# ArchieGertsman/spark-sched-sim

Hardware: AMD Instinct MI355X
Metric: env-steps/sec at 4096 batched envs (TPC-H, 10 exec) (higher is better)
Workload: dtype int64+f64

## Files before the change

include/sss.h:

```cpp
#ifndef SSS_H
#define SSS_H
#include <stddef.h>
#include <stdint.h>

#ifdef __cplusplus
extern "C" {
#endif

typedef struct sss_handle sss_handle;

typedef struct sss_cfg {
  int32_t num_executors;
  int32_t job_arrival_cap;
  int32_t max_jobs;
  int32_t reserved;
  double job_arrival_rate;
  double moving_delay;
  double warmup_delay;
  double beta;
} sss_cfg;

typedef struct sss_dims {
  int32_t num_envs, num_executors, job_cap, stage_stride;
  int32_t node_cap;
// ... 24 lines not shown
  SSS_E_STALLED = 5,
  SSS_E_NO_DURATION = 6,
  SSS_E_INVARIANT = 7,
  SSS_E_NEED_RESET = 8,
  SSS_E_NO_LIMIT = 9,
  SSS_E_CAPACITY = 10
};

int sss_query_dims(const sss_cfg* cfg, const void* pack, size_t pack_bytes, int num_envs, sss_dims* out);

int sss_create(const sss_cfg* cfg, const void* pack, size_t pack_bytes, int num_envs, int device, sss_handle** out);

int sss_bind_buffers(sss_handle* h, const sss_buffers* buffers);

int sss_reset(sss_handle* h, const uint64_t* seeds_dev, const double* time_limits_dev, const uint8_t* mask_dev, void* stream);

#define SSS_SKIP_ENV (-2147483647 - 1)
int sss_step(sss_handle* h, const int32_t* stage_idx_dev, const int32_t* num_exec_dev, int auto_reset, uint64_t seed_stride, void* stream);

int sss_step_bounded(sss_handle* h, const int32_t* stage_idx_dev, const int32_t* num_exec_dev, int auto_reset, uint64_t seed_stride, int max_events,
                     uint8_t* ready_dev, void* stream);

int sss_policy(sss_handle* h, int policy, int param, int32_t* stage_idx_dev, int32_t* num_exec_dev, void* stream);

int sss_rollout(sss_handle* h, int policy, int param, int n_steps, int auto_reset, uint64_t seed_stride, void* stream);

typedef struct sss_decima_graph {
  const uint8_t* active_dev;
  const int64_t* node_off_dev;
  const int64_t* job_off_dev;
  const int64_t* edge_off_dev;
  float num_tasks_scale;
  float work_scale;
  float* x_dev;
  int64_t* node_obs_dev;
  int64_t* node_loc_dev;
  int64_t* node_job_dev;
  int64_t* sched_rank_dev;
  int32_t* gen_dev;
  uint32_t* node_recv_dev;
  uint8_t* stage_mask_dev;
  int64_t* src_dev;
  int64_t* dst_dev;
  int64_t* edge_obs_dev;
  uint32_t* edge_layers_dev;
  int64_t* job_obs_dev;
// ... 378 lines not shown
```

spark_sched_sim_amd/binding.py:

```python
from __future__ import annotations

import ctypes as C
import os.path as osp

CSRC = osp.join(osp.dirname(osp.abspath(__file__)), "csrc")
LIB_NAME = "libsss_hip.so"


class SssCfg(C.Structure):
    _fields_ = [("num_executors", C.c_int32), ("job_arrival_cap", C.c_int32), ("max_jobs", C.c_int32),
                ("reserved", C.c_int32), ("job_arrival_rate", C.c_double), ("moving_delay", C.c_double),
                ("warmup_delay", C.c_double), ("beta", C.c_double)]


class SssDims(C.Structure):
    _fields_ = [("num_envs", C.c_int32), ("num_executors", C.c_int32), ("job_cap", C.c_int32),
                ("stage_stride", C.c_int32), ("node_cap", C.c_int32), ("edge_cap", C.c_int32),
                ("obs_i32", C.c_int32), ("obs_f64", C.c_int32), ("state_bytes", C.c_int64),
                ("env_stride", C.c_int64), ("off_t_arrival", C.c_int64), ("off_t_completed", C.c_int64),
                ("off_jobs", C.c_int64), ("off_active", C.c_int64), ("off_dur_ring", C.c_int64),
                ("job_rec_bytes", C.c_int32), ("hdr_bytes", C.c_int32)]


class SssBuffers(C.Structure):
# ... 133 lines not shown
    _fields_ = [("t_dev", C.c_void_p), ("job_dev", C.c_void_p), ("count_dev", C.c_void_p), ("cap", C.c_int32), ("pad_", C.c_int32)]


class SssTimelineRenderArgs(C.Structure):
    _fields_ = [("env_ids_dev", C.c_void_p), ("n", C.c_int32), ("width", C.c_int32), ("height", C.c_int32), ("pad_", C.c_int32), ("rgb_dev", C.c_void_p)]


REWARD_WINDOW_CHUNK = 64


def reward_window_scratch(T: int, B: int) -> int:
    return ((T + REWARD_WINDOW_CHUNK - 1) // REWARD_WINDOW_CHUNK + 1) * B + 1


class SssArenaArray(C.Structure):
    _fields_ = [("src_dev", C.c_void_p), ("dst_dev", C.c_void_p), ("elem_bytes", C.c_int32), ("per_row", C.c_int32), ("kind", C.c_int32), ("shift", C.c_int32)]


class SssArenaArgs(C.Structure):
    _fields_ = [("n_arrays", C.c_int32), ("n_obs", C.c_int32), ("totals_dev", C.c_void_p), ("cursor_dev", C.c_void_p), ("capacity", C.c_int64 * 4),
                ("rows_hint", C.c_int64), ("arrays", SssArenaArray * 24)]


EXPORTS = ["sss_query_dims", "sss_create", "sss_bind_buffers", "sss_reset", "sss_step", "sss_step_bounded", "sss_policy", "sss_rollout",
           "sss_decima_graph_build", "sss_decima_layer_lists", "sss_prefix_rows", "sss_decima_policy", "sss_decima_sample", "sss_gnn_launch",
           "sss_linear_wgrad_scratch", "sss_linear_wgrad", "sss_mlp_supported", "sss_mlp_recompute_supported", "sss_mlp_split_supported", "sss_mlp_forward", "sss_mlp_backward", "sss_mlp_wgrad_scratch", "sss_mlp_backward_wgrad", "sss_mlp_wgrad_finish", "sss_collect_step", "sss_gnn_encode", "sss_rows_op", "sss_rows_concat", "sss_segment_categorical", "sss_bit_lists", "sss_arena_append", "sss_discounted_returns", "sss_sequence_baselines", "sss_reward_window_update", "sss_differential_returns", "sss_bind_timeline", "sss_timeline_render", "sss_last_error", "sss_destroy", "sss_abi_sizeof"]
POLICY_IDS = {"fair": 0, "fifo": 1, "hash": 2, "wfair": 3, "sjfcp": 4}
WFAIR_ALPHA_RANGE = (-4, 4)
ABI_STRUCTS = {"sss_cfg": SssCfg, "sss_dims": SssDims, "sss_buffers": SssBuffers, "sss_decima_graph": SssDecimaGraph, "sss_decima_lists": SssDecimaLists,
               "sss_bit_list_args": SssBitListArgs, "sss_gnn_args": SssGnnArgs, "sss_decima_policy_args": SssDecimaPolicyArgs,
               "sss_decima_sample_args": SssDecimaSampleArgs, "sss_gnn_encode_args": SssGnnEncodeArgs, "sss_collect_args": SssCollectArgs,
               "sss_mlp_args": SssMlpArgs, "sss_arena_array": SssArenaArray, "sss_arena_args": SssArenaArgs, "sss_returns_args": SssReturnsArgs,
               "sss_baseline_args": SssBaselineArgs, "sss_rows_args": SssRowsArgs, "sss_concat_part": SssConcatPart, "sss_concat_args": SssConcatArgs, "sss_segcat_args": SssSegcatArgs}
ABI_TAGGED_STRUCTS = {"sss_reward_window_args": SssRewardWindowArgs, "sss_diffret_args": SssDiffretArgs}
ABI_PLAIN_STRUCTS = {"sss_timeline": SssTimeline, "sss_timeline_render_args": SssTimelineRenderArgs}


def load_library(path: str | None = None) -> C.CDLL:
    path = path or osp.join(CSRC, LIB_NAME)
    if not osp.exists(path):
        raise RuntimeError(
            f"{path} not found: the HIP extension has not been built "
            "(run `python -c 'import __graft_entry__ as g; g.build()'` or spark_sched_sim_amd/build.py). "
            "There is no CPU fallback.")
    return C.CDLL(path)


class Binding:
    def __init__(self, lib: C.CDLL | None = None):
        self.lib = lib if lib is not None else load_library()
        L = self.lib
        L.sss_query_dims.argtypes = [C.POINTER(SssCfg), C.c_void_p, C.c_size_t, C.c_int, C.POINTER(SssDims)]
        L.sss_create.argtypes = [C.POINTER(SssCfg), C.c_void_p, C.c_size_t, C.c_int, C.c_int, C.POINTER(C.c_void_p)]
        L.sss_bind_buffers.argtypes = [C.c_void_p, C.POINTER(SssBuffers)]
        L.sss_reset.argtypes = [C.c_void_p, C.c_void_p, C.c_void_p, C.c_void_p, C.c_void_p]
        L.sss_step.argtypes = [C.c_void_p, C.c_void_p, C.c_void_p, C.c_int, C.c_uint64, C.c_void_p]
        L.sss_step_bounded.argtypes = [C.c_void_p, C.c_void_p, C.c_void_p, C.c_int, C.c_uint64, C.c_int, C.c_void_p, C.c_void_p]
        L.sss_policy.argtypes = [C.c_void_p, C.c_int, C.c_int, C.c_void_p, C.c_void_p, C.c_void_p]
        L.sss_rollout.argtypes = [C.c_void_p, C.c_int, C.c_int, C.c_int, C.c_int, C.c_uint64, C.c_void_p]
        L.sss_decima_graph_build.argtypes = [C.c_void_p, C.POINTER(SssDecimaGraph), C.c_void_p]
        L.sss_decima_layer_lists.argtypes = [C.c_int, C.POINTER(SssDecimaLists), C.c_void_p]
        L.sss_prefix_rows.argtypes = [C.c_void_p, C.c_int64, C.c_int64, C.c_void_p, C.c_int, C.c_int, C.c_void_p, C.c_void_p, C.c_void_p, C.c_void_p]
        L.sss_decima_policy.argtypes = [C.c_void_p, C.POINTER(SssDecimaPolicyArgs), C.c_void_p]
        L.sss_decima_sample.argtypes = [C.c_int, C.c_int, C.POINTER(SssDecimaSampleArgs), C.c_void_p]
        L.sss_gnn_launch.argtypes = [C.c_int, C.POINTER(SssGnnArgs), C.c_void_p]
        L.sss_linear_wgrad_scratch.argtypes = [C.c_int, C.c_int]
        L.sss_linear_wgrad_scratch.restype = C.c_int64
        L.sss_linear_wgrad.argtypes = [C.c_void_p, C.c_int64, C.c_void_p, C.c_int64, C.c_int64, C.c_int, C.c_int, C.c_void_p, C.c_void_p, C.c_void_p, C.c_void_p]
        L.sss_gnn_encode.argtypes = [C.POINTER(SssGnnEncodeArgs), C.c_void_p]
        L.sss_collect_step.argtypes = [C.POINTER(SssCollectArgs), C.c_int, C.c_void_p]
        L.sss_mlp_supported.argtypes = [C.c_int] * 5
        L.sss_mlp_recompute_supported.argtypes = [C.c_int]
        L.sss_mlp_split_supported.argtypes = [C.c_int]
        L.sss_mlp_forward.argtypes = [C.POINTER(SssMlpArgs), C.c_void_p]
        L.sss_mlp_backward.argtypes = [C.POINTER(SssMlpArgs), C.c_void_p]
        L.sss_mlp_wgrad_scratch.argtypes = [C.c_int]
        L.sss_mlp_wgrad_scratch.restype = C.c_int64
        L.sss_mlp_backward_wgrad.argtypes = [C.POINTER(SssMlpArgs), C.c_void_p, C.c_void_p]
        L.sss_mlp_wgrad_finish.argtypes = [C.c_int] + [C.c_void_p] * 8
        L.sss_discounted_returns.argtypes = [C.POINTER(SssReturnsArgs), C.c_void_p]
# ... 43 lines not shown
```

spark_sched_sim_amd/csrc/sss_hip_sim.hip:

```cpp
#include <hip/hip_runtime.h>

#include "sss_sim.h"
#include "sss_narrow.h"

#ifdef SSS_TIMELINE
#define SSS_LAUNCHER(name) sss_narrow_tl_launch_##name
#define SSS_TL_DISPATCH(call)
#else
#define SSS_LAUNCHER(name) sss_narrow_launch_##name
#define SSS_TL_DISPATCH(call) \
  if (a.tl.t) return sss_narrow_tl_launch_##call
int sss_narrow_hot_bytes() { return (int)sizeof(SssHot); }
int sss_narrow_static_lds_bytes() { return SSS_STATIC_LDS_BYTES; }
#endif

int SSS_LAUNCHER(reset)(const SssKernelArgs& a, int num_envs, const uint64_t* seeds, const double* tl, const uint8_t* mask, void* stream) {
  SSS_TL_DISPATCH(reset(a, num_envs, seeds, tl, mask, stream));
  hipLaunchKernelGGL(SSS_KNAME(sss_reset_kernel), dim3(num_envs), dim3(64), (size_t)a.P.pool_bytes, (hipStream_t)stream, a, seeds, tl, mask);
  return (int)hipGetLastError();
}
int SSS_LAUNCHER(step_bounded)(const SssKernelArgs& a, int num_envs, const int32_t* stage_idx, const int32_t* num_exec, int auto_reset, uint64_t seed_stride,
                                   int budget, uint8_t* ready, void* stream) {
  SSS_TL_DISPATCH(step_bounded(a, num_envs, stage_idx, num_exec, auto_reset, seed_stride, budget, ready, stream));
  hipLaunchKernelGGL(SSS_KNAME(sss_step_bounded_kernel), dim3(num_envs), dim3(64), (size_t)a.P.pool_bytes, (hipStream_t)stream, a, stage_idx, num_exec, auto_reset, seed_stride,
                     budget, ready);
  return (int)hipGetLastError();
}
int SSS_LAUNCHER(step)(const SssKernelArgs& a, int num_envs, const int32_t* stage_idx, const int32_t* num_exec, int auto_reset, uint64_t seed_stride,
                           void* stream) {
  SSS_TL_DISPATCH(step(a, num_envs, stage_idx, num_exec, auto_reset, seed_stride, stream));
  hipLaunchKernelGGL(SSS_KNAME(sss_step_kernel), dim3(num_envs), dim3(64), (size_t)a.P.pool_bytes, (hipStream_t)stream, a, stage_idx, num_exec, auto_reset, seed_stride);
  return (int)hipGetLastError();
}
#ifndef SSS_TIMELINE
int SSS_LAUNCHER(policy)(const SssKernelArgs& a, int num_envs, int policy, int param, int32_t* stage_idx, int32_t* num_exec, void* stream) {
  hipLaunchKernelGGL(SSS_KNAME(sss_policy_kernel), dim3(num_envs), dim3(64), (size_t)a.P.pool_bytes, (hipStream_t)stream, a, policy, param, stage_idx, num_exec);
  return (int)hipGetLastError();
}
#endif
int SSS_LAUNCHER(rollout)(const SssKernelArgs& a, int num_envs, int policy, int param, int n_steps, int auto_reset, uint64_t seed_stride, void* stream) {
  SSS_TL_DISPATCH(rollout(a, num_envs, policy, param, n_steps, auto_reset, seed_stride, stream));
  if (policy >= SSS_POLICY_WFAIR)
    hipLaunchKernelGGL(SSS_KNAME(sss_rollout_heur_kernel), dim3(num_envs), dim3(64), (size_t)a.P.pool_bytes, (hipStream_t)stream, a, policy, param, n_steps, auto_reset, seed_stride);
  else
    hipLaunchKernelGGL(SSS_KNAME(sss_rollout_kernel), dim3(num_envs), dim3(64), (size_t)a.P.pool_bytes, (hipStream_t)stream, a, policy, param, n_steps, auto_reset, seed_stride);
  return (int)hipGetLastError();
}

#if defined(SSS_EVPROF3) && !defined(SSS_TIMELINE)
extern "C" int sss_debug_prof(unsigned long long* out64) {
  if (hipMemcpyFromSymbol(out64, HIP_SYMBOL(g_prof3), sizeof(unsigned long long) * 96) != hipSuccess) return -1;
  static const unsigned long long zeros[96] = {0};
  return hipMemcpyToSymbol(HIP_SYMBOL(g_prof3), zeros, sizeof(zeros)) == hipSuccess ? 0 : -1;
// ... 6 lines not shown
```

spark_sched_sim_amd/csrc/sss_hip_wide.hip:

```cpp
#define SSS_WIDE 1
#include <hip/hip_runtime.h>

#include "sss_sim.h"
#include "sss_wide.h"

#ifdef SSS_TIMELINE
#define SSS_LAUNCHER(name) sss_wide_tl_launch_##name
#define SSS_TL_DISPATCH(call)
#else
#define SSS_LAUNCHER(name) sss_wide_launch_##name
#define SSS_TL_DISPATCH(call) \
  if (a.tl.t) return sss_wide_tl_launch_##call
int sss_wide_hot_bytes() { return (int)sizeof(SssHot); }
int sss_wide_static_lds_bytes() { return SSS_STATIC_LDS_BYTES; }
#endif

int SSS_LAUNCHER(reset)(const SssKernelArgs& a, int num_envs, const uint64_t* seeds, const double* tl, const uint8_t* mask, void* stream) {
  SSS_TL_DISPATCH(reset(a, num_envs, seeds, tl, mask, stream));
  hipLaunchKernelGGL(SSS_KNAME(sss_reset_kernel), dim3(num_envs), dim3(64), (size_t)a.P.pool_bytes, (hipStream_t)stream, a, seeds, tl, mask);
  return (int)hipGetLastError();
}
int SSS_LAUNCHER(step_bounded)(const SssKernelArgs& a, int num_envs, const int32_t* stage_idx, const int32_t* num_exec, int auto_reset, uint64_t seed_stride,
                                 int budget, uint8_t* ready, void* stream) {
  SSS_TL_DISPATCH(step_bounded(a, num_envs, stage_idx, num_exec, auto_reset, seed_stride, budget, ready, stream));
  hipLaunchKernelGGL(SSS_KNAME(sss_step_bounded_kernel), dim3(num_envs), dim3(64), (size_t)a.P.pool_bytes, (hipStream_t)stream, a, stage_idx, num_exec, auto_reset,
                     seed_stride, budget, ready);
  return (int)hipGetLastError();
}
int SSS_LAUNCHER(step)(const SssKernelArgs& a, int num_envs, const int32_t* stage_idx, const int32_t* num_exec, int auto_reset, uint64_t seed_stride,
                         void* stream) {
  SSS_TL_DISPATCH(step(a, num_envs, stage_idx, num_exec, auto_reset, seed_stride, stream));
  hipLaunchKernelGGL(SSS_KNAME(sss_step_kernel), dim3(num_envs), dim3(64), (size_t)a.P.pool_bytes, (hipStream_t)stream, a, stage_idx, num_exec, auto_reset, seed_stride);
  return (int)hipGetLastError();
}
#ifndef SSS_TIMELINE
int SSS_LAUNCHER(policy)(const SssKernelArgs& a, int num_envs, int policy, int param, int32_t* stage_idx, int32_t* num_exec, void* stream) {
  hipLaunchKernelGGL(SSS_KNAME(sss_policy_kernel), dim3(num_envs), dim3(64), (size_t)a.P.pool_bytes, (hipStream_t)stream, a, policy, param, stage_idx, num_exec);
  return (int)hipGetLastError();
}
#endif
int SSS_LAUNCHER(rollout)(const SssKernelArgs& a, int num_envs, int policy, int param, int n_steps, int auto_reset, uint64_t seed_stride, void* stream) {
  SSS_TL_DISPATCH(rollout(a, num_envs, policy, param, n_steps, auto_reset, seed_stride, stream));
  if (policy >= SSS_POLICY_WFAIR)
    hipLaunchKernelGGL(SSS_KNAME(sss_rollout_heur_kernel), dim3(num_envs), dim3(64), (size_t)a.P.pool_bytes, (hipStream_t)stream, a, policy, param, n_steps, auto_reset, seed_stride);
  else
    hipLaunchKernelGGL(SSS_KNAME(sss_rollout_kernel), dim3(num_envs), dim3(64), (size_t)a.P.pool_bytes, (hipStream_t)stream, a, policy, param, n_steps, auto_reset, seed_stride);
  return (int)hipGetLastError();
}

#if defined(SSS_EVPROF3) && !defined(SSS_TIMELINE)
extern "C" int sss_debug_prof_wide(unsigned long long* out64) {
  if (hipMemcpyFromSymbol(out64, HIP_SYMBOL(g_prof3), sizeof(unsigned long long) * 96) != hipSuccess) return -1;
  static const unsigned long long zeros[96] = {0};
  return hipMemcpyToSymbol(HIP_SYMBOL(g_prof3), zeros, sizeof(zeros)) == hipSuccess ? 0 : -1;
// ... 6 lines not shown
```

spark_sched_sim_amd/csrc/sss_host.h:

```cpp
#pragma once
#include <math.h>
#include <stdio.h>
#include <stdlib.h>
#include <string.h>

#include <string>
#include <vector>

#include "../../include/sss.h"
#include "sss_layout.h"
#include "sss_train.h"
#include "sss_rows.h"
#include "sss_narrow.h"
#include "sss_wide.h"
#include "sss_timeline.h"

static bool sss_is_wide(int num_executors) { return num_executors > 64; }
static int sss_hot_bytes(int num_executors) { return sss_is_wide(num_executors) ? sss_wide_hot_bytes() : sss_narrow_hot_bytes(); }

static thread_local std::string g_sss_err;
static int sss_fail(int code, const std::string& msg) {
  g_sss_err = msg;
  return code;
}
// ... 360 lines not shown
  pk.pcg_jump = (const uint64_t*)h->jump_dev;
  pk.lvl_thr = (const uint64_t*)h->jump_dev + jump_words;
  pk.common_pool = (const uint8_t*)h->common_dev;
  h->pk = pk;
  *out = h;
  return 0;
}

extern "C" int sss_bind_buffers(sss_handle* h, const sss_buffers* b) {
  if (!h || !b) return sss_fail(-1, "NULL argument");
  if (!b->state_dev || !b->nodes_dev || !b->edge_links_dev || !b->dag_ptr_dev || !b->exec_supplies_dev || !b->obs_i32_dev || !b->obs_f64_dev)
    return sss_fail(-20, "every buffer in sss_buffers must be provided");
  if (((uintptr_t)b->state_dev) & 255) return sss_fail(-21, "state_dev must be 256-byte aligned");
  h->B.state = b->state_dev, h->B.nodes = b->nodes_dev, h->B.edge_links = b->edge_links_dev, h->B.dag_ptr = b->dag_ptr_dev;
  h->B.exec_supplies = b->exec_supplies_dev, h->B.obs_i32 = b->obs_i32_dev, h->B.obs_f64 = b->obs_f64_dev;
  h->B.gen = h->bound ? h->B.gen + 1 : 1, h->B.gen_pad = 0;
  h->bound = true;
  return 0;
}

static SssKernelArgs sss_args(const sss_handle* h) {
  SssKernelArgs a;
  a.L = h->L, a.B = h->B, a.P = h->P, a.pk = h->pk, a.tl = h->tl;
  return a;
}

extern "C" int sss_bind_timeline(sss_handle* h, const struct sss_timeline* tl) {
  if (!h) return sss_fail(-1, "NULL argument");
  if (!tl) {
    memset(&h->tl, 0, sizeof(h->tl));
    return 0;
  }
  if (!tl->t_dev) return sss_fail(-40, "sss_bind_timeline: t_dev is NULL");
  if (!tl->job_dev) return sss_fail(-40, "sss_bind_timeline: job_dev is NULL");
  if (!tl->count_dev) return sss_fail(-40, "sss_bind_timeline: count_dev is NULL");
  if (tl->cap < 1) return sss_fail(-40, "sss_bind_timeline: cap must be >= 1, got " + std::to_string(tl->cap));
  h->tl.t = tl->t_dev, h->tl.job = tl->job_dev, h->tl.count = tl->count_dev, h->tl.cap = tl->cap, h->tl.pad_ = 0;
  return 0;
}

extern "C" int sss_timeline_render(sss_handle* h, const struct sss_timeline_render_args* a, void* stream) {
  if (!h || !a) return sss_fail(-1, "NULL argument");
  if (!h->bound) return sss_fail(-22, "sss_bind_buffers has not been called");
  if (!h->tl.t) return sss_fail(-41, "sss_timeline_render: no timeline is bound (sss_bind_timeline)");
  if (a->n < 0 || a->n > h->L.num_envs) return sss_fail(-41, "sss_timeline_render: n must be in 0..num_envs");
  if (a->width < 1 || a->width > 16384 || a->height < 1 || a->height > 16384) return sss_fail(-41, "sss_timeline_render: width and height must be in 1..16384");
// ... 36 lines not shown
  if (max_events < 1) return sss_fail(-35, "sss_step_bounded: max_events must be at least 1");
  BeDeviceGuard guard(h->device);
  const SssKernelArgs ka = sss_args(h);
  if (int rc = sss_is_wide(h->L.E) ? sss_wide_launch_step_bounded(ka, h->L.num_envs, stage_idx_dev, num_exec_dev, auto_reset, seed_stride, max_events, ready_dev, stream)
                                   : be_launch_step_bounded(ka, h->L.num_envs, stage_idx_dev, num_exec_dev, auto_reset, seed_stride, max_events, ready_dev, stream))
    return sss_fail(-30, std::string("step launch failed: ") + be_error(rc));
  return 0;
}

static int sss_check_policy(int policy, int param) {
  if (policy < 0 || policy > 4) return sss_fail(-23, "unknown policy");
  if (policy == 3 && (param < -4 || param > 4)) return sss_fail(-23, "weighted fair: alpha (param) must be in [-4, 4], got " + std::to_string(param));
  return 0;
}

extern "C" int sss_policy(sss_handle* h, int policy, int param, int32_t* stage_idx_dev, int32_t* num_exec_dev, void* stream) {
  if (!h || !stage_idx_dev || !num_exec_dev) return sss_fail(-1, "NULL argument");
  if (!h->bound) return sss_fail(-22, "sss_bind_buffers has not been called");
  BeDeviceGuard guard(h->device);
  if (int rc = sss_check_policy(policy, param)) return rc;
  const SssKernelArgs ka = sss_args(h);
  if (int rc = sss_is_wide(h->L.E) ? sss_wide_launch_policy(ka, h->L.num_envs, policy, param, stage_idx_dev, num_exec_dev, stream)
                                   : be_launch_policy(ka, h->L.num_envs, policy, param, stage_idx_dev, num_exec_dev, stream)) return sss_fail(-30, std::string("policy launch failed: ") + be_error(rc));
  return 0;
}

extern "C" int sss_rollout(sss_handle* h, int policy, int param, int n_steps, int auto_reset, uint64_t seed_stride, void* stream) {
  if (!h) return sss_fail(-1, "NULL argument");
  if (!h->bound) return sss_fail(-22, "sss_bind_buffers has not been called");
  BeDeviceGuard guard(h->device);
  if (int rc = sss_check_policy(policy, param)) return rc;
  if (n_steps < 0) return sss_fail(-24, "n_steps must be >= 0");
  const SssKernelArgs ka = sss_args(h);
  if (int rc = sss_is_wide(h->L.E) ? sss_wide_launch_rollout(ka, h->L.num_envs, policy, param, n_steps, auto_reset, seed_stride, stream)
                                   : be_launch_rollout(ka, h->L.num_envs, policy, param, n_steps, auto_reset, seed_stride, stream)) return sss_fail(-30, std::string("rollout launch failed: ") + be_error(rc));
  return 0;
}

extern "C" int sss_decima_graph_build(sss_handle* h, const sss_decima_graph* g, void* stream) {
  if (!h || !g) return sss_fail(-1, "NULL argument");
  if (!h->bound) return sss_fail(-22, "sss_bind_buffers has not been called");
  BeDeviceGuard guard(h->device);
  if (!g->node_off_dev || !g->job_off_dev || !g->edge_off_dev || !g->x_dev || !g->node_obs_dev || !g->node_loc_dev || !g->node_job_dev ||
      !g->sched_rank_dev || !g->gen_dev || !g->node_recv_dev || !g->stage_mask_dev || !g->src_dev || !g->dst_dev || !g->edge_obs_dev ||
      !g->edge_layers_dev || !g->job_obs_dev || !g->job_cap_dev || !g->job_first_dev || !g->obs_depth_dev ||
      !g->job_nodes_dev || !g->out_start_dev || !g->out_deg_dev || !g->layer_cnt_dev)
// ... 465 lines not shown
```

spark_sched_sim_amd/csrc/sss_layout.h:

```cpp
#pragma once
#include <stdint.h>

#ifdef SSS_WIDE
#define SSS_MAX_EXEC 128
#else
#define SSS_MAX_EXEC 64
#endif
#define SSS_MAX_EXEC_ANY 128
#define SSS_MAX_STAGES 64
#define SSS_MAX_JOBS 1024
#define SSS_JOBSET_SLOTS 2048
#define SSS_MAX_LEVELS 16
#ifdef SSS_WIDE
#define SSS_SET_TABLE 1024
#else
#define SSS_SET_TABLE 256
#endif
#define sss_pool_table_bytes_any(E) ((E) >= 128 ? 1024 : ((E) >= 64 ? 512 : 256))
#ifdef SSS_WIDE
#define sss_pool_table_bytes(E) ((E) >= 128 ? 1024 : 512)
#else
#define sss_pool_table_bytes(E) ((E) >= 64 ? 512 : 256)
#endif
#define SSS_DUR_RING 200
// ... 156 lines not shown
  const uint8_t* common_pool;
  const uint64_t* pcg_jump;
  const uint64_t* lvl_thr;
};

struct SssBuffers {
  void* state;
  float* nodes;
  int32_t* edge_links;
  int32_t* dag_ptr;
  int32_t* exec_supplies;
  int32_t* obs_i32;
  double* obs_f64;
  uint32_t gen, gen_pad;
};

struct SssTimeline {
  double* t;
  int32_t* job;
  int32_t* count;
  int32_t cap, pad_;
};

struct SssKernelArgs {
  SssLayout L;
  SssBuffers B;
  SssParams P;
  SssPackDev pk;
  SssTimeline tl;
};

static inline int64_t sss_align(int64_t x, int64_t a) { return (x + a - 1) / a * a; }

#define SSS_LDS_BUDGET 10240

struct SssExDesc {
  int32_t gs;
  int8_t li, ri;
  int16_t thr_n;
  int32_t off_l, lenw_l;
  uint32_t thr_lo, thr_hi;
  int32_t off_r, lenw_r;
};

static inline int sss_compute_lds_pool(SssParams* P, int J_cap, int SP, int E, int static_bytes) {
  int jobset = J_cap <= 76 ? 128 : (J_cap <= 306 ? 512 : 2048);
  int o = 0;
  P->off_active = o, o += 2 * J_cap;
  P->off_old_active = o, o += 2 * J_cap;
  P->off_slot_of = o, o += J_cap;
  P->off_slot_ref = o, o += 64;
  o = (o + 1) & ~1;
// ... 52 lines not shown
```

spark_sched_sim_amd/csrc/sss_sim.h:

```cpp
#pragma once
#ifdef SSS_WIDE
#ifdef SSS_TIMELINE
#define SSS_KNAME(name) name##_wide_tl
#else
#define SSS_KNAME(name) name##_wide
#endif
#else
#ifdef SSS_TIMELINE
#define SSS_KNAME(name) name##_tl
#else
#define SSS_KNAME(name) name
#endif
#endif
#include "../../include/sss.h"
#include "sss_layout.h"
#include <wave_rt.h>


struct alignas(16) SssScratch {
  uint8_t pool8[8];
  uint8_t pool8b[8];
  uint64_t rng_buf[64];
  int32_t rng_pos, pad0_[3];
  uint8_t setA[SSS_SET_TABLE];
// ... 269 lines not shown
#include "sss_sim_tracker.h"
#include "sss_sim_jobs.h"
#include "sss_sim_fulfil.h"
#include "sss_sim_events.h"
#include "sss_sim_fast_run.h"
#include "sss_sim_batches.h"
#include "sss_sim_lean.h"
#include "sss_sim_observe.h"
#include "sss_sim_env.h"
#undef SSS_SRC_ID
#define SSS_SRC_ID 0

SSS_KERNEL void SSS_KNAME(sss_reset_kernel)(SssKernelArgs a, const uint64_t* seeds, const double* time_limits, const uint8_t* mask) {
  int env = wave_env();
  if (mask && !mask[env]) return;
  uint8_t* base = (uint8_t*)a.B.state + (size_t)env * a.L.env_stride;
  ctx_init();
  env_begin(base);
  do_reset(a.L, seeds[env], time_limits ? time_limits[env] : __builtin_inf());
  write_observation(a.L, a.B, env, 0.0);
  env_end(base);
}

SSS_DEV void step_env(const SssKernelArgs& a, const int32_t* stage_idx, const int32_t* num_exec, int auto_reset, uint64_t seed_stride, int budget, uint8_t* ready) {
  int env = wave_env();
  if (stage_idx[env] == SSS_SKIP_ENV) return;
  uint8_t* base = (uint8_t*)a.B.state + (size_t)env * a.L.env_stride;
  ctx_init();
  env_begin(base);
  double reward = 0.0;
  bool yielded = false;
  bool start_next_episode = wave_ballot(auto_reset && g_hot.h.terminated && !g_hot.h.err) != 0;
  if (start_next_episode) {
    do_reset(a.L, g_hot.h.seed + seed_stride, g_hot.h.time_limit);
  } else {
    reward = do_step(stage_idx[env], num_exec[env], budget, &yielded);
  }
  if (!yielded) write_observation(a.L, a.B, env, reward);
  if (ready && wave_lane() == 0) ready[env] = yielded ? 0 : 1;
  env_end(base);
  prof3_flush();
}
SSS_KERNEL void SSS_KNAME(sss_step_kernel)(SssKernelArgs a, const int32_t* stage_idx, const int32_t* num_exec, int auto_reset, uint64_t seed_stride) {
  step_env(a, stage_idx, num_exec, auto_reset, seed_stride, 0, nullptr);
}
SSS_KERNEL void SSS_KNAME(sss_step_bounded_kernel)(SssKernelArgs a, const int32_t* stage_idx, const int32_t* num_exec, int auto_reset, uint64_t seed_stride,
                                                   int budget, uint8_t* ready) {
  step_env(a, stage_idx, num_exec, auto_reset, seed_stride, budget, ready);
}


SSS_DEV int obs_num_committable() {
  uint32_t srck = g_hot.h.curr_source;
  if (srck == POOL_NONE) return 0;
  int p = pool_index(srck);
  return (int)g_c.pool_hdr[p].used - (int)g_c.pool_hdr[p].commit_from;
}

SSS_DEV int find_stage_dev(uint64_t sm, uint64_t act, int gs) {
  int best = -1;
  uint64_t m = sm;
  while (m) {
    int s = ctz64(m);
    m &= m - 1;
    if ((g_c.pk.stage_parent_mask[gs + s] & act) == 0) {
      best = s;
      break;
    }
  }
  if (best < 0 && sm) best = ctz64(sm);
  return best;
// ... 199 lines not shown
  x += 0x9E3779B97F4A7C15ull;
  uint64_t z = x;
  z = (z ^ (z >> 30)) * 0xBF58476D1CE4E5B9ull;
  z = (z ^ (z >> 27)) * 0x94D049BB133111EBull;
  return z ^ (z >> 31);
}

SSS_DEV void policy_hash(int p_none_permille, int& stage_idx, int& num_exec) {
  uint64_t seed = g_hot.h.seed;
  uint64_t step = (uint64_t)g_hot.h.ep_steps;
  int n_sched = g_hot.h.n_sched;
  int ncommit = obs_num_committable();
  wave_sync();
  uint64_t h = splitmix64((seed << 32) ^ step), h2 = splitmix64(h), h3 = splitmix64(h2);
  if (n_sched == 0 || (int)(h3 % 1000) < p_none_permille)
    stage_idx = -1;
  else
    stage_idx = (int)(h % (uint64_t)n_sched);
  num_exec = 1 + (int)(h2 % (uint64_t)(ncommit > 0 ? ncommit : 1));
}

enum { SSS_POLICY_FAIR = 0, SSS_POLICY_FIFO = 1, SSS_POLICY_HASH = 2, SSS_POLICY_WFAIR = 3, SSS_POLICY_SJFCP = 4 };

template <bool kHeuristics = true>
SSS_DEV void run_policy(int policy, int param, int& stage_idx, int& num_exec) {
  PROF3(29);
  if (policy == SSS_POLICY_HASH)
    policy_hash(param, stage_idx, num_exec);
  else if (kHeuristics && policy == SSS_POLICY_WFAIR)
    policy_wfair(param, stage_idx, num_exec);
  else if (kHeuristics && policy == SSS_POLICY_SJFCP)
    policy_sjfcp(stage_idx, num_exec);
  else
    policy_fair(policy == SSS_POLICY_FAIR, stage_idx, num_exec);
}

#ifndef SSS_TIMELINE
SSS_KERNEL void SSS_KNAME(sss_policy_kernel)(SssKernelArgs a, int policy, int param, int32_t* stage_idx, int32_t* num_exec) {
  int env = wave_env();
  uint8_t* base = (uint8_t*)a.B.state + (size_t)env * a.L.env_stride;
  ctx_init();
  env_begin_readonly(base);
  int si, ne;
  run_policy(policy, param, si, ne);
  if (wave_lane() == 0) stage_idx[env] = si, num_exec[env] = ne;
}
#endif

#define ROLLOUT_BODY(kHeuristics) \
  int env = wave_env(); \
  uint8_t* base = (uint8_t*)a.B.state + (size_t)env * a.L.env_stride; \
  ctx_init(); \
  env_begin(base); \
  for (int it = 0; it < n_steps; it++) { \
    bool over = wave_ballot(g_hot.h.terminated || g_hot.h.need_reset) != 0; \
    double reward = 0.0; \
    if (over) { \
      if (!auto_reset || wave_ballot(g_hot.h.err != 0) != 0) break;  \
      do_reset(a.L, g_hot.h.seed + seed_stride, g_hot.h.time_limit); \
    } else { \
      int si, ne; \
      run_policy<kHeuristics>(policy, param, si, ne); \
      reward = do_step<true>(si, ne); \
    } \
    write_observation(a.L, a.B, env, reward); \
    wave_sync(); \
  } \
// ... 23 lines not shown
```

spark_sched_sim_amd/vec_env.py:

```python
from __future__ import annotations

import ctypes as C
from typing import Any, Sequence

import numpy as np
import torch

from . import workload
from .binding import (ERROR_NAMES, POLICY_IDS, WFAIR_ALPHA_RANGE, Binding, SssBuffers, SssCfg, SssDecimaGraph, SssDecimaLists, SssTimeline,
                      SssTimelineRenderArgs, device_of)

OBS_FIELDS = ("n_nodes", "n_edges", "n_jobs", "n_schedulable", "num_committable_execs", "source_job_idx",
              "terminated", "err")
NUM_NODE_FEATURES = 3


class BatchedObs(dict):
    """dict of device tensors; rows beyond n_nodes[i] / n_edges[i] / n_jobs[i] of env i are padding.

    keys: nodes f32[B, node_cap, 3], edge_links i32[B, edge_cap, 2], dag_ptr i32[B, job_cap+1],
    exec_supplies i32[B, job_cap], plus one i32[B] tensor per OBS_FIELDS entry.
    """


# ... 35 lines not shown
        self.bufs[k].copy_(t, non_blocking=True)
        if self.cuda:
            self.events[k].record(torch.cuda.current_stream(t.device))
        self.posted[k], self.last, self.tags[k] = True, k, tag


class VecSparkSchedSimEnv:

    def __init__(self, env_cfg: dict[str, Any], num_envs: int, device: str | torch.device = "cuda:0",
                 pack: bytes | None = None, auto_reset: bool = False, seed_stride: int | None = None,
                 _lib: C.CDLL | None = None) -> None:
        self.device = torch.device(device)
        if self.device.type != "cuda" and _lib is None:
            raise RuntimeError("VecSparkSchedSimEnv runs on an AMD GPU (device='cuda:N'); there is no CPU path")
        sampler = env_cfg.get("data_sampler_cls", "TPCHDataSampler")
        if sampler != "TPCHDataSampler":
            raise ValueError(f"'{sampler}' is not a valid data sampler.")
        self.num_envs = int(num_envs)
        self.num_executors = int(env_cfg["num_executors"])
        self.env_cfg = dict(env_cfg)
        self.auto_reset = bool(auto_reset)
        self.seed_stride = int(seed_stride if seed_stride is not None else num_envs)
        self._b = Binding(_lib)
        self._pack = pack if pack is not None else workload.default_pack()
        cap = env_cfg.get("job_arrival_cap")
        self._cfg = SssCfg(self.num_executors, int(cap) if cap else 0, int(env_cfg.get("max_jobs") or 0), 0,
                           float(env_cfg["job_arrival_rate"]), float(env_cfg["moving_delay"]),
                           float(env_cfg["warmup_delay"]), float(env_cfg.get("beta", 0.0)))
        self.dims = self._b.query_dims(self._cfg, self._pack, self.num_envs)
        dev_index = self.device.index or 0
        self._h = self._b.create(self._cfg, self._pack, self.num_envs, dev_index if self.device.type == "cuda" else -1)
        d, B, dev = self.dims, self.num_envs, self.device
        self._state_raw = torch.zeros(d.state_bytes + 256, dtype=torch.uint8, device=dev)
        off = (-self._state_raw.data_ptr()) % 256
        self.state = self._state_raw[off: off + d.state_bytes]
        self.nodes = torch.zeros((B, d.node_cap, NUM_NODE_FEATURES), dtype=torch.float32, device=dev)
        self.edge_links = torch.zeros((B, d.edge_cap, 2), dtype=torch.int32, device=dev)
        self.dag_ptr = torch.zeros((B, d.job_cap + 1), dtype=torch.int32, device=dev)
        self.exec_supplies = torch.zeros((B, d.job_cap), dtype=torch.int32, device=dev)
        self.obs_i32 = torch.zeros((B, d.obs_i32), dtype=torch.int32, device=dev)
        self.obs_f64 = torch.zeros((B, d.obs_f64), dtype=torch.float64, device=dev)
        self.rebind_buffers()
        self._seeds = torch.zeros(B, dtype=torch.int64, device=dev)
        self._tl = torch.full((B,), float("inf"), dtype=torch.float64, device=dev)
        self._mask = torch.ones(B, dtype=torch.uint8, device=dev)
        self._env_view = self.state.view(B, d.env_stride)
        self._act_stage = torch.zeros(B, dtype=torch.int32, device=dev)
        self._act_nexec = torch.ones(B, dtype=torch.int32, device=dev)
        self._closed = False
        self._dg_pool: dict[int, torch.Tensor] = {}
        self._layer_scratch: dict = {}
        self._never = None
        from .workload import pack_max_depth
        self.max_dag_depth = pack_max_depth(self._pack)
        from .spaces import make_action_space, make_observation_space
        self.single_action_space = make_action_space(self.num_executors)
        self.action_space = self.single_action_space
        self.single_observation_space = make_observation_space(self.num_executors, NUM_NODE_FEATURES)
        self.observation_space = self.single_observation_space


    def rebind_buffers(self) -> None:
        bufs = SssBuffers(self.state.data_ptr(), self.nodes.data_ptr(), self.edge_links.data_ptr(),
                          self.dag_ptr.data_ptr(), self.exec_supplies.data_ptr(), self.obs_i32.data_ptr(),
                          self.obs_f64.data_ptr())
        self._b.check(self._b.lib.sss_bind_buffers(self._h, C.byref(bufs)))
        self._bind_timeline()

    def _stream(self) -> int:
        return torch.cuda.current_stream(self.device).cuda_stream if self.device.type == "cuda" else 0

    def _obs(self) -> BatchedObs:
        o = BatchedObs(nodes=self.nodes, edge_links=self.edge_links, dag_ptr=self.dag_ptr,
                       exec_supplies=self.exec_supplies)
        for k, name in enumerate(OBS_FIELDS):
            o[name] = self.obs_i32[:, k]
        return o

    def close(self) -> None:
        if not self._closed:
            if self.device.type == "cuda":
                torch.cuda.synchronize(self.device)
            self._b.lib.sss_destroy(self._h)
            self._closed = True

    def __del__(self):
        try:
            self.close()
        except Exception:
            pass


    def reset(self, *, seed: int | Sequence[int] | None = None, options: dict[str, Any] | None = None,
              mask: torch.Tensor | None = None):
        B = self.num_envs
        if seed is None:
            seeds = np.random.SeedSequence().generate_state(B, np.uint64) >> np.uint64(1)
        elif isinstance(seed, (int, np.integer)):
            seeds = np.arange(B, dtype=np.uint64) + np.uint64(int(seed))
        else:
            seeds = np.asarray(list(seed), dtype=np.uint64)
            if seeds.shape != (B,):
                raise ValueError("need one seed per env")
        self._seeds.copy_(torch.from_numpy(seeds.view(np.int64)))
        tl = (options or {}).get("time_limit", np.inf)
        tl_arr = np.broadcast_to(np.asarray(tl, dtype=np.float64), (B,)).copy()
        self._tl.copy_(torch.from_numpy(tl_arr))
        mask_ptr = None
        if mask is not None:
            self._mask.copy_(mask.to(torch.uint8))
            mask_ptr = self._mask.data_ptr()
        self._b.check(self._b.lib.sss_reset(self._h, self._seeds.data_ptr(), self._tl.data_ptr(), mask_ptr, self._stream()))
        return self._obs(), {"wall_time": self.obs_f64[:, 1]}

    def step_async(self, stage_idx: torch.Tensor, num_exec: torch.Tensor) -> None:
        assert stage_idx.dtype == torch.int32 and num_exec.dtype == torch.int32
        assert stage_idx.device == self.device and stage_idx.is_contiguous() and num_exec.is_contiguous()
        self._b.check(self._b.lib.sss_step(self._h, stage_idx.data_ptr(), num_exec.data_ptr(), int(self.auto_reset),
                                           self.seed_stride, self._stream()))

    def step_bounded_async(self, stage_idx: torch.Tensor, num_exec: torch.Tensor, max_events: int, ready: torch.Tensor | None = None) -> torch.Tensor:
        assert stage_idx.dtype == torch.int32 and num_exec.dtype == torch.int32
        assert stage_idx.device == self.device and stage_idx.is_contiguous() and num_exec.is_contiguous()
        if ready is None:
            if getattr(self, "_ready", None) is None:
                self._ready = torch.ones(self.num_envs, dtype=torch.uint8, device=self.device)
            ready = self._ready
        assert ready.dtype == torch.uint8 and ready.is_contiguous() and ready.numel() == self.num_envs
        self._b.check(self._b.lib.sss_step_bounded(self._h, stage_idx.data_ptr(), num_exec.data_ptr(), int(self.auto_reset), self.seed_stride, int(max_events),
                                                   ready.data_ptr(), self._stream()))
        return ready

    def step(self, actions):
        if set(actions.keys()) != {"stage_idx", "num_exec"}:
            raise ValueError("invalid action: does not belong to the action space")
        self.step_async(actions["stage_idx"], actions["num_exec"])
        obs = self._obs()
        f64 = self.obs_f64.clone()
        i32 = self.obs_i32[:, 6:8].clone()
        terminated = i32[:, 0] != 0
        if self._never is None or self._never.shape != terminated.shape:
            self._never = torch.zeros_like(terminated)
        return obs, f64[:, 0], terminated, self._never, {"wall_time": f64[:, 1], "err": i32[:, 1]}


    def _bind_timeline(self) -> None:
        tl = getattr(self, "_timeline", None)
        if tl is None:
            self._b.check(self._b.lib.sss_bind_timeline(self._h, None))
            return
        t, job, count = tl
        a = SssTimeline(t.data_ptr(), job.data_ptr(), count.data_ptr(), t.shape[2], 0)
        self._b.check(self._b.lib.sss_bind_timeline(self._h, C.byref(a)))

    def enable_timeline(self, cap: int = 256) -> None:
        cap = int(cap)
        if cap < 1:
            raise ValueError(f"enable_timeline: cap must be >= 1, got {cap}")
        B, E, dev = self.num_envs, self.num_executors, self.device
        t = torch.full((B, E, cap), float("nan"), dtype=torch.float64, device=dev)
        job = torch.full((B, E, cap), -1, dtype=torch.int32, device=dev)
        count = torch.ones((B, E), dtype=torch.int32, device=dev)
        self._timeline = (t, job, count)
        self._bind_timeline()

    def disable_timeline(self) -> None:
        self._timeline = None
        self._bind_timeline()

    def timeline_arrays(self) -> tuple[torch.Tensor, torch.Tensor, torch.Tensor]:
# ... 17 lines not shown
        if env_ids is None:
            ids, n = None, self.num_envs
        else:
            ids = torch.as_tensor(env_ids, dtype=torch.int32).reshape(-1).to(dev).contiguous()
            n = int(ids.numel())
            if n and (int(ids.min()) < 0 or int(ids.max()) >= self.num_envs):
                raise IndexError("render: env id out of range")
        rgb = torch.empty((n, int(height), int(width), 3), dtype=torch.uint8, device=dev)
        a = SssTimelineRenderArgs(ids.data_ptr() if ids is not None and n else None, n, int(width), int(height), 0, rgb.data_ptr() if n else None)
        self._b.check(self._b.lib.sss_timeline_render(self._h, C.byref(a), self._stream()))
        return rgb


    @staticmethod
    def _policy_id(policy: str, param: int) -> int:
        pid = POLICY_IDS[policy]
        lo, hi = WFAIR_ALPHA_RANGE
        if policy == "wfair" and not lo <= int(param) <= hi:
            raise ValueError(f"wfair: alpha (param) must be an integer in [{lo}, {hi}], got {param}")
        return pid

    def policy_actions(self, policy: str = "fair", param: int = 0):
        pid = self._policy_id(policy, param)
        self._b.check(self._b.lib.sss_policy(self._h, pid, int(param), self._act_stage.data_ptr(),
                                             self._act_nexec.data_ptr(), self._stream()))
        return {"stage_idx": self._act_stage, "num_exec": self._act_nexec}

    def rollout(self, policy: str, n_steps: int, param: int = 0) -> None:
        pid = self._policy_id(policy, param)
        self._b.check(self._b.lib.sss_rollout(self._h, pid, int(param), int(n_steps), int(self.auto_reset),
                                              self.seed_stride, self._stream()))

    def decima_graph_on_device(self, active: torch.Tensor | None = None, num_tasks_scale: float = 200.0, work_scale: float = 1e5) -> dict[str, Any]:
        B, dev, d = self.num_envs, self.device, self.dims
        assert self.graph_kernel_fits, "the graph kernel's LDS working set does not fit this node capacity"
        D = self.max_dag_depth
        ws = getattr(self, "_dg_dev", None)
        if ws is None:
            Mc, Ec, Jc = B * d.node_cap, B * d.edge_cap, B * d.job_cap
            e = lambda n, dt, *tail: torch.empty((max(n, 1), *tail), dtype=dt, device=dev)
            ws = self._dg_dev = {
                "x": e(Mc, torch.float32, 5), "node_obs": e(Mc, torch.int64), "node_loc": e(Mc, torch.int64), "node_job": e(Mc, torch.int64),
                "sched_rank": e(Mc, torch.int64), "gen": e(Mc, torch.int32), "node_recv": e(Mc, torch.int32), "stage_mask": e(Mc, torch.bool),
                "src": e(Ec, torch.int64), "dst": e(Ec, torch.int64), "edge_obs": e(Ec, torch.int64), "edge_layers": e(Ec, torch.int32),
                "job_obs": e(Jc, torch.int64), "job_cap": e(Jc, torch.int64), "job_first": e(Jc, torch.int64), "obs_depth": e(B, torch.int32),
                "job_nodes": e(Jc, torch.int64), "out_start": e(Mc, torch.int64), "out_deg": e(Mc, torch.int32),
                "layer_cnt": e(32, torch.int32, B), "sched_list": e(Mc, torch.int64),
                "scan": e(2, torch.int64, 4, B),
                "pp": torch.zeros(1056 + 4 + 1056, dtype=torch.int64, device=dev),
                "recv": e(Mc * max(D, 1), torch.int64), "hint": LateHint(1060, dev), "epoch": 0}
            ws["tot"] = ws["pp"][1056:1060]
        act8 = _mask_u8(active)
# ... 251 lines not shown
```

Before: 24.06 million.

## Fold heuristic policy evaluation into the step kernel with prefetched double-buffered actions

Adds a fused step+policy kernel: after a step, the step kernel computes the next heuristic policy action (fair/fifo/hash) while the env state is still in LDS and writes it to a double-buffered action pair. When policy_actions is then called with the same policy and unchanged tensors, the Python side swaps buffers instead of launching a separate policy kernel. This removes one kernel launch and a re-read of env state per step in the policy-driven loop, at the cost of more bookkeeping using tensor version checks and a larger kernel-args struct.

```diff
diff --git a/include/sss.h b/include/sss.h
--- a/include/sss.h
+++ b/include/sss.h
@@ -70,6 +70,9 @@
                      uint8_t* ready_dev, void* stream);
 
 int sss_policy(sss_handle* h, int policy, int param, int32_t* stage_idx_dev, int32_t* num_exec_dev, void* stream);
+
+int sss_step_policy(sss_handle* h, const int32_t* stage_idx_dev, const int32_t* num_exec_dev, int auto_reset, uint64_t seed_stride, int policy, int param,
+                    int32_t* next_stage_idx_dev, int32_t* next_num_exec_dev, int* folded, void* stream);
 
 int sss_rollout(sss_handle* h, int policy, int param, int n_steps, int auto_reset, uint64_t seed_stride, void* stream);
 
diff --git a/spark_sched_sim_amd/binding.py b/spark_sched_sim_amd/binding.py
--- a/spark_sched_sim_amd/binding.py
+++ b/spark_sched_sim_amd/binding.py
@@ -179,9 +179,11 @@
                 ("rows_hint", C.c_int64), ("arrays", SssArenaArray * 24)]
 
 
-EXPORTS = ["sss_query_dims", "sss_create", "sss_bind_buffers", "sss_reset", "sss_step", "sss_step_bounded", "sss_policy", "sss_rollout",
+EXPORTS = ["sss_query_dims", "sss_create", "sss_bind_buffers", "sss_reset", "sss_step", "sss_step_bounded", "sss_step_policy", "sss_policy", "sss_rollout",
            "sss_decima_graph_build", "sss_decima_layer_lists", "sss_prefix_rows", "sss_decima_policy", "sss_decima_sample", "sss_gnn_launch",
            "sss_linear_wgrad_scratch", "sss_linear_wgrad", "sss_mlp_supported", "sss_mlp_recompute_supported", "sss_mlp_split_supported", "sss_mlp_forward", "sss_mlp_backward", "sss_mlp_wgrad_scratch", "sss_mlp_backward_wgrad", "sss_mlp_wgrad_finish", "sss_collect_step", "sss_gnn_encode", "sss_rows_op", "sss_rows_concat", "sss_segment_categorical", "sss_bit_lists", "sss_arena_append", "sss_discounted_returns", "sss_sequence_baselines", "sss_reward_window_update", "sss_differential_returns", "sss_bind_timeline", "sss_timeline_render", "sss_last_error", "sss_destroy", "sss_abi_sizeof"]
+HANDLE_READERS = frozenset({"sss_policy", "sss_decima_graph_build", "sss_decima_policy", "sss_timeline_render", "sss_destroy"})
+HANDLE_STATE_CHANGING = frozenset({"sss_bind_buffers", "sss_reset", "sss_step", "sss_step_bounded", "sss_step_policy", "sss_rollout", "sss_bind_timeline"})
 POLICY_IDS = {"fair": 0, "fifo": 1, "hash": 2, "wfair": 3, "sjfcp": 4}
 WFAIR_ALPHA_RANGE = (-4, 4)
 ABI_STRUCTS = {"sss_cfg": SssCfg, "sss_dims": SssDims, "sss_buffers": SssBuffers, "sss_decima_graph": SssDecimaGraph, "sss_decima_lists": SssDecimaLists,
@@ -213,6 +215,7 @@
         L.sss_reset.argtypes = [C.c_void_p, C.c_void_p, C.c_void_p, C.c_void_p, C.c_void_p]
         L.sss_step.argtypes = [C.c_void_p, C.c_void_p, C.c_void_p, C.c_int, C.c_uint64, C.c_void_p]
         L.sss_step_bounded.argtypes = [C.c_void_p, C.c_void_p, C.c_void_p, C.c_int, C.c_uint64, C.c_int, C.c_void_p, C.c_void_p]
+        L.sss_step_policy.argtypes = [C.c_void_p, C.c_void_p, C.c_void_p, C.c_int, C.c_uint64, C.c_int, C.c_int, C.c_void_p, C.c_void_p, C.POINTER(C.c_int), C.c_void_p]
         L.sss_policy.argtypes = [C.c_void_p, C.c_int, C.c_int, C.c_void_p, C.c_void_p, C.c_void_p]
         L.sss_rollout.argtypes = [C.c_void_p, C.c_int, C.c_int, C.c_int, C.c_int, C.c_uint64, C.c_void_p]
         L.sss_decima_graph_build.argtypes = [C.c_void_p, C.POINTER(SssDecimaGraph), C.c_void_p]
diff --git a/spark_sched_sim_amd/csrc/sss_hip_sim.hip b/spark_sched_sim_amd/csrc/sss_hip_sim.hip
--- a/spark_sched_sim_amd/csrc/sss_hip_sim.hip
+++ b/spark_sched_sim_amd/csrc/sss_hip_sim.hip
@@ -29,6 +29,12 @@
 int SSS_LAUNCHER(step)(const SssKernelArgs& a, int num_envs, const int32_t* stage_idx, const int32_t* num_exec, int auto_reset, uint64_t seed_stride,
                            void* stream) {
   SSS_TL_DISPATCH(step(a, num_envs, stage_idx, num_exec, auto_reset, seed_stride, stream));
+#ifndef SSS_TIMELINE
+  if (a.fold.fold_policy >= 0) {
+    hipLaunchKernelGGL(SSS_KNAME(sss_step_policy_kernel), dim3(num_envs), dim3(64), (size_t)a.P.pool_bytes, (hipStream_t)stream, a, stage_idx, num_exec, auto_reset, seed_stride);
+    return (int)hipGetLastError();
+  }
+#endif
   hipLaunchKernelGGL(SSS_KNAME(sss_step_kernel), dim3(num_envs), dim3(64), (size_t)a.P.pool_bytes, (hipStream_t)stream, a, stage_idx, num_exec, auto_reset, seed_stride);
   return (int)hipGetLastError();
 }
diff --git a/spark_sched_sim_amd/csrc/sss_hip_wide.hip b/spark_sched_sim_amd/csrc/sss_hip_wide.hip
--- a/spark_sched_sim_amd/csrc/sss_hip_wide.hip
+++ b/spark_sched_sim_amd/csrc/sss_hip_wide.hip
@@ -30,6 +30,12 @@
 int SSS_LAUNCHER(step)(const SssKernelArgs& a, int num_envs, const int32_t* stage_idx, const int32_t* num_exec, int auto_reset, uint64_t seed_stride,
                          void* stream) {
   SSS_TL_DISPATCH(step(a, num_envs, stage_idx, num_exec, auto_reset, seed_stride, stream));
+#ifndef SSS_TIMELINE
+  if (a.fold.fold_policy >= 0) {
+    hipLaunchKernelGGL(SSS_KNAME(sss_step_policy_kernel), dim3(num_envs), dim3(64), (size_t)a.P.pool_bytes, (hipStream_t)stream, a, stage_idx, num_exec, auto_reset, seed_stride);
+    return (int)hipGetLastError();
+  }
+#endif
   hipLaunchKernelGGL(SSS_KNAME(sss_step_kernel), dim3(num_envs), dim3(64), (size_t)a.P.pool_bytes, (hipStream_t)stream, a, stage_idx, num_exec, auto_reset, seed_stride);
   return (int)hipGetLastError();
 }
diff --git a/spark_sched_sim_amd/csrc/sss_host.h b/spark_sched_sim_amd/csrc/sss_host.h
--- a/spark_sched_sim_amd/csrc/sss_host.h
+++ b/spark_sched_sim_amd/csrc/sss_host.h
@@ -406,6 +406,7 @@
 static SssKernelArgs sss_args(const sss_handle* h) {
   SssKernelArgs a;
   a.L = h->L, a.B = h->B, a.P = h->P, a.pk = h->pk, a.tl = h->tl;
+  a.fold.fold_policy = -1, a.fold.fold_param = 0, a.fold.next_stage_idx = nullptr, a.fold.next_num_exec = nullptr;
   return a;
 }
 
@@ -488,6 +489,26 @@
   const SssKernelArgs ka = sss_args(h);
   if (int rc = sss_is_wide(h->L.E) ? sss_wide_launch_policy(ka, h->L.num_envs, policy, param, stage_idx_dev, num_exec_dev, stream)
                                    : be_launch_policy(ka, h->L.num_envs, policy, param, stage_idx_dev, num_exec_dev, stream)) return sss_fail(-30, std::string("policy launch failed: ") + be_error(rc));
+  return 0;
+}
+
+extern "C" int sss_step_policy(sss_handle* h, const int32_t* stage_idx_dev, const int32_t* num_exec_dev, int auto_reset, uint64_t seed_stride, int policy, int param,
+                               int32_t* next_stage_idx_dev, int32_t* next_num_exec_dev, int* folded, void* stream) {
+  if (!h || !stage_idx_dev || !num_exec_dev || !next_stage_idx_dev || !next_num_exec_dev) return sss_fail(-1, "NULL argument");
+  if (!h->bound) return sss_fail(-22, "sss_bind_buffers has not been called");
+  if (int rc = sss_check_policy(policy, param)) return rc;
+  const bool wide = sss_is_wide(h->L.E);
+  const bool fold = policy <= 2 && !h->tl.t;
+  if (folded) *folded = fold ? 1 : 0;
+  if (!fold) {
+    if (int rc = sss_step(h, stage_idx_dev, num_exec_dev, auto_reset, seed_stride, stream)) return rc;
+    return sss_policy(h, policy, param, next_stage_idx_dev, next_num_exec_dev, stream);
+  }
+  BeDeviceGuard guard(h->device);
+  SssKernelArgs ka = sss_args(h);
+  ka.fold.fold_policy = policy, ka.fold.fold_param = param, ka.fold.next_stage_idx = next_stage_idx_dev, ka.fold.next_num_exec = next_num_exec_dev;
+  if (int rc = wide ? sss_wide_launch_step(ka, h->L.num_envs, stage_idx_dev, num_exec_dev, auto_reset, seed_stride, stream)
+                    : be_launch_step(ka, h->L.num_envs, stage_idx_dev, num_exec_dev, auto_reset, seed_stride, stream)) return sss_fail(-30, std::string("step launch failed: ") + be_error(rc));
   return 0;
 }
 
diff --git a/spark_sched_sim_amd/csrc/sss_layout.h b/spark_sched_sim_amd/csrc/sss_layout.h
--- a/spark_sched_sim_amd/csrc/sss_layout.h
+++ b/spark_sched_sim_amd/csrc/sss_layout.h
@@ -202,12 +202,19 @@
   int32_t cap, pad_;
 };
 
+struct SssFold {
+  int32_t fold_policy, fold_param;
+  int32_t* next_stage_idx;
+  int32_t* next_num_exec;
+};
+
 struct SssKernelArgs {
   SssLayout L;
   SssBuffers B;
   SssParams P;
   SssPackDev pk;
   SssTimeline tl;
+  SssFold fold;
 };
 
 static inline int64_t sss_align(int64_t x, int64_t a) { return (x + a - 1) / a * a; }
diff --git a/spark_sched_sim_amd/csrc/sss_sim.h b/spark_sched_sim_amd/csrc/sss_sim.h
--- a/spark_sched_sim_amd/csrc/sss_sim.h
+++ b/spark_sched_sim_amd/csrc/sss_sim.h
@@ -315,31 +315,63 @@
   env_end(base);
 }
 
+template <bool kHeuristics>
+SSS_DEV void run_policy(int policy, int param, int& stage_idx, int& num_exec);
+SSS_DEV bool fold_on() { return ((const SssKernelArgs*)SSS_KERNARG_PTR())->fold.fold_policy >= 0; }
+SSS_DEV void fold_policy_store(int env) {
+  const SssKernelArgs* a = (const SssKernelArgs*)SSS_KERNARG_PTR();
+  int si, ne;
+  run_policy<false>(a->fold.fold_policy, a->fold.fold_param, si, ne);
+  if (wave_lane() == 0) a->fold.next_stage_idx[env] = si, a->fold.next_num_exec[env] = ne;
+}
+
+template <bool FOLD>
 SSS_DEV void step_env(const SssKernelArgs& a, const int32_t* stage_idx, const int32_t* num_exec, int auto_reset, uint64_t seed_stride, int budget, uint8_t* ready) {
   int env = wave_env();
-  if (stage_idx[env] == SSS_SKIP_ENV) return;
+  const bool skip = stage_idx[env] == SSS_SKIP_ENV;
+  if (skip && !(FOLD && fold_on())) return;
   uint8_t* base = (uint8_t*)a.B.state + (size_t)env * a.L.env_stride;
   ctx_init();
-  env_begin(base);
-  double reward = 0.0;
-  bool yielded = false;
-  bool start_next_episode = wave_ballot(auto_reset && g_hot.h.terminated && !g_hot.h.err) != 0;
-  if (start_next_episode) {
-    do_reset(a.L, g_hot.h.seed + seed_stride, g_hot.h.time_limit);
+  if (FOLD && skip) {
+    env_begin_readonly(base);
   } else {
-    reward = do_step(stage_idx[env], num_exec[env], budget, &yielded);
-  }
-  if (!yielded) write_observation(a.L, a.B, env, reward);
-  if (ready && wave_lane() == 0) ready[env] = yielded ? 0 : 1;
+    env_begin(base);
+    double reward = 0.0;
+    bool yielded = false;
+    bool start_next_episode = wave_ballot(auto_reset && g_hot.h.terminated && !g_hot.h.err) != 0;
+    if (start_next_episode) {
+      do_reset(a.L, g_hot.h.seed + seed_stride, g_hot.h.time_limit);
+    } else {
+      reward = do_step(stage_idx[env], num_exec[env], budget, &yielded);
+    }
+    if (!yielded) write_observation(a.L, a.B, env, reward);
+    if (ready && wave_lane() == 0) ready[env] = yielded ? 0 : 1;
+  }
+  if (FOLD && fold_on()) {
+    wave_sync();
+    fold_policy_store(env);
+  }
+  if (FOLD && skip) return;
   env_end(base);
   prof3_flush();
 }
+#if defined(__HIP__)
+#define SSS_STEP_FOLDS false
+#else
+#define SSS_STEP_FOLDS true
+#endif
 SSS_KERNEL void SSS_KNAME(sss_step_kernel)(SssKernelArgs a, const int32_t* stage_idx, const int32_t* num_exec, int auto_reset, uint64_t seed_stride) {
-  step_env(a, stage_idx, num_exec, auto_reset, seed_stride, 0, nullptr);
-}
+  step_env<SSS_STEP_FOLDS>(a, stage_idx, num_exec, auto_reset, seed_stride, 0, nullptr);
+}
+#if defined(__HIP__) && !defined(SSS_TIMELINE)
+SSS_KERNEL void SSS_KNAME(sss_step_policy_kernel)(SssKernelArgs a, const int32_t* stage_idx, const int32_t* num_exec, int auto_reset, uint64_t seed_stride) {
+  step_env<true>(a, stage_idx, num_exec, auto_reset, seed_stride, 0, nullptr);
+}
+#endif
+#undef SSS_STEP_FOLDS
 SSS_KERNEL void SSS_KNAME(sss_step_bounded_kernel)(SssKernelArgs a, const int32_t* stage_idx, const int32_t* num_exec, int auto_reset, uint64_t seed_stride,
                                                    int budget, uint8_t* ready) {
-  step_env(a, stage_idx, num_exec, auto_reset, seed_stride, budget, ready);
+  step_env<false>(a, stage_idx, num_exec, auto_reset, seed_stride, budget, ready);
 }
 
 
@@ -585,7 +617,7 @@
 
 enum { SSS_POLICY_FAIR = 0, SSS_POLICY_FIFO = 1, SSS_POLICY_HASH = 2, SSS_POLICY_WFAIR = 3, SSS_POLICY_SJFCP = 4 };
 
-template <bool kHeuristics = true>
+template <bool kHeuristics>
 SSS_DEV void run_policy(int policy, int param, int& stage_idx, int& num_exec) {
   PROF3(29);
   if (policy == SSS_POLICY_HASH)
@@ -605,7 +637,7 @@
   ctx_init();
   env_begin_readonly(base);
   int si, ne;
-  run_policy(policy, param, si, ne);
+  run_policy<true>(policy, param, si, ne);
   if (wave_lane() == 0) stage_idx[env] = si, num_exec[env] = ne;
 }
 #endif
diff --git a/spark_sched_sim_amd/vec_env.py b/spark_sched_sim_amd/vec_env.py
--- a/spark_sched_sim_amd/vec_env.py
+++ b/spark_sched_sim_amd/vec_env.py
@@ -81,6 +81,7 @@
         self.auto_reset = bool(auto_reset)
         self.seed_stride = int(seed_stride if seed_stride is not None else num_envs)
         self._b = Binding(_lib)
+        self._issued = self._prefetch = None
         self._pack = pack if pack is not None else workload.default_pack()
         cap = env_cfg.get("job_arrival_cap")
         self._cfg = SssCfg(self.num_executors, int(cap) if cap else 0, int(env_cfg.get("max_jobs") or 0), 0,
@@ -104,8 +105,10 @@
         self._tl = torch.full((B,), float("inf"), dtype=torch.float64, device=dev)
         self._mask = torch.ones(B, dtype=torch.uint8, device=dev)
         self._env_view = self.state.view(B, d.env_stride)
-        self._act_stage = torch.zeros(B, dtype=torch.int32, device=dev)
-        self._act_nexec = torch.ones(B, dtype=torch.int32, device=dev)
+        self._act_pairs = [(torch.zeros(B, dtype=torch.int32, device=dev), torch.ones(B, dtype=torch.int32, device=dev)) for _ in range(2)]
+        self._act_cur = 0
+        self._act_stage, self._act_nexec = self._act_pairs[0]
+        self._tracks_versions = not any(t.is_inference() for t in (self._state_raw, *self._act_pairs[0], *self._act_pairs[1]))
         self._closed = False
         self._dg_pool: dict[int, torch.Tensor] = {}
         self._layer_scratch: dict = {}
@@ -123,8 +126,12 @@
         bufs = SssBuffers(self.state.data_ptr(), self.nodes.data_ptr(), self.edge_links.data_ptr(),
                           self.dag_ptr.data_ptr(), self.exec_supplies.data_ptr(), self.obs_i32.data_ptr(),
                           self.obs_f64.data_ptr())
+        self._drop_prefetch()
         self._b.check(self._b.lib.sss_bind_buffers(self._h, C.byref(bufs)))
         self._bind_timeline()
+
+    def _drop_prefetch(self) -> None:
+        self._issued = self._prefetch = None
 
     def _stream(self) -> int:
         return torch.cuda.current_stream(self.device).cuda_stream if self.device.type == "cuda" else 0
@@ -169,14 +176,27 @@
         if mask is not None:
             self._mask.copy_(mask.to(torch.uint8))
             mask_ptr = self._mask.data_ptr()
+        self._drop_prefetch()
         self._b.check(self._b.lib.sss_reset(self._h, self._seeds.data_ptr(), self._tl.data_ptr(), mask_ptr, self._stream()))
         return self._obs(), {"wall_time": self.obs_f64[:, 1]}
 
     def step_async(self, stage_idx: torch.Tensor, num_exec: torch.Tensor) -> None:
         assert stage_idx.dtype == torch.int32 and num_exec.dtype == torch.int32
         assert stage_idx.device == self.device and stage_idx.is_contiguous() and num_exec.is_contiguous()
-        self._b.check(self._b.lib.sss_step(self._h, stage_idx.data_ptr(), num_exec.data_ptr(), int(self.auto_reset),
-                                           self.seed_stride, self._stream()))
+        issued, stream = self._issued, self._stream()
+        if issued is None or not self._tracks_versions or stage_idx is not self._act_stage or num_exec is not self._act_nexec:
+            self._drop_prefetch()
+            self._b.check(self._b.lib.sss_step(self._h, stage_idx.data_ptr(), num_exec.data_ptr(), int(self.auto_reset), self.seed_stride, stream))
+            return
+        nxt = self._act_pairs[1 - self._act_cur]
+        folded = C.c_int(0)
+        self._prefetch = None
+        self._b.check(self._b.lib.sss_step_policy(self._h, stage_idx.data_ptr(), num_exec.data_ptr(), int(self.auto_reset), self.seed_stride, issued[0], issued[1],
+                                                  nxt[0].data_ptr(), nxt[1].data_ptr(), C.byref(folded), stream))
+        self._prefetch = (issued, stream, self._prefetch_versions())
+
+    def _prefetch_versions(self) -> tuple:
+        return (self.state._version,) + tuple(t._version for pair in self._act_pairs for t in pair)
 
     def step_bounded_async(self, stage_idx: torch.Tensor, num_exec: torch.Tensor, max_events: int, ready: torch.Tensor | None = None) -> torch.Tensor:
         assert stage_idx.dtype == torch.int32 and num_exec.dtype == torch.int32
@@ -186,6 +206,7 @@
                 self._ready = torch.ones(self.num_envs, dtype=torch.uint8, device=self.device)
             ready = self._ready
         assert ready.dtype == torch.uint8 and ready.is_contiguous() and ready.numel() == self.num_envs
+        self._drop_prefetch()
         self._b.check(self._b.lib.sss_step_bounded(self._h, stage_idx.data_ptr(), num_exec.data_ptr(), int(self.auto_reset), self.seed_stride, int(max_events),
                                                    ready.data_ptr(), self._stream()))
         return ready
@@ -205,6 +226,7 @@
 
     def _bind_timeline(self) -> None:
         tl = getattr(self, "_timeline", None)
+        self._drop_prefetch()
         if tl is None:
             self._b.check(self._b.lib.sss_bind_timeline(self._h, None))
             return
@@ -268,12 +290,18 @@
 
     def policy_actions(self, policy: str = "fair", param: int = 0):
         pid = self._policy_id(policy, param)
-        self._b.check(self._b.lib.sss_policy(self._h, pid, int(param), self._act_stage.data_ptr(),
-                                             self._act_nexec.data_ptr(), self._stream()))
+        key, stream, pf = (pid, int(param)), self._stream(), self._prefetch
+        if pf is not None and pf[0] == key and pf[1] == stream and pf[2] == self._prefetch_versions():
+            self._act_cur ^= 1
+            self._act_stage, self._act_nexec = self._act_pairs[self._act_cur]
+        else:
+            self._b.check(self._b.lib.sss_policy(self._h, pid, int(param), self._act_stage.data_ptr(), self._act_nexec.data_ptr(), stream))
+        self._prefetch, self._issued = None, key
         return {"stage_idx": self._act_stage, "num_exec": self._act_nexec}
 
     def rollout(self, policy: str, n_steps: int, param: int = 0) -> None:
         pid = self._policy_id(policy, param)
+        self._drop_prefetch()
         self._b.check(self._b.lib.sss_rollout(self._h, pid, int(param), int(n_steps), int(self.auto_reset),
                                               self.seed_stride, self._stream()))
 
```

New measurement: 24.26 million (median of 6 runs). Within noise of the previous version (+0.8%).
